# Advaith-Sajeev/LiDAR-Vision-VQA

Measured on AMD Instinct MI355X. Metric: fused tokens/sec/GPU + cross-attn MFMA-roofline % (32k pts x 196 patches), higher is better.
Workload: dtype bf16; 1 GPU; BASELINE configs[1]: 32768-pt scenes (Dist-C) -> hard voxelise (0.1, 0.1, 0.2) T=10 max=60000 + MeanVFE; pillars (0.2, 0.2, 8.0) T=20 max=30000 -> PillarVFE[64] -> PointPillarScatter 512x512 (as an index map; sparse key stream: K|V computed only for the cells with a pillar in their 3x3 neighbourhood, by LayerNorm and the K|V projection folded onto the 64-channel conv token, every other key from th; parallelism=scene-parallel x1

## Files before the change

include/lvq.h:

```cpp
#ifndef LVQ_H
#define LVQ_H

#include <stddef.h>
#include <stdint.h>

#ifdef __cplusplus
extern "C" {
#endif

typedef void *lvq_stream_t;
typedef uint16_t lvq_bf16;

enum {
    LVQ_OK = 0,
    LVQ_EINVAL = -1,
    LVQ_EWORKSPACE = -2,
    LVQ_ELAUNCH = -3,
    LVQ_EOVERFLOW = -4,
    LVQ_EUNSUPPORTED = -5
};

const char *lvq_version(void);
const char *lvq_strerror(int code);

typedef struct lvq_tuning {
    int32_t attn_no32;
    int32_t attn32_nw;
    int32_t attn_pipe;
    int32_t attn_nsplit;
    int32_t attn_qt;
    int32_t attn_nw;
    int32_t gemm_no_gemv;
    int32_t gemm_stream_c_mb;
    int32_t gemm_no256;
    int32_t gemm_no256x256;
    int32_t gemm_256x256_min_tiles;
    int32_t gemm_ln_tiles;
    int32_t pillar_vfe_generic;
    int32_t voxel_path;
    int32_t pairs_one_wg;
    int32_t ca_fused_variant;
    uint64_t ca_fused_stamps;
    int32_t conv_rows_grid;
    int32_t reserved[7];
} lvq_tuning;
void lvq_tuning_defaults(lvq_tuning *t);
int lvq_set_tuning(const lvq_tuning *t);
int lvq_get_tuning(lvq_tuning *t);


int lvq_mask_points_by_range(const float *pts, int64_t n, int c, const float *range_host, uint8_t *keep,
                             lvq_stream_t stream);

size_t lvq_voxelize_hard_workspace_bytes(int64_t n_points, int n_scenes);
int lvq_voxelize_hard(const float *pts, const int32_t *scene_off, int64_t n_points, int n_scenes, int c,
                      const float *range_host, const float *vsize_host, const int32_t *grid_host,
                      int max_pts, int max_voxels, int break_on_cap, int64_t voxel_capacity,
                      float *voxels, int32_t *coords_bzyx, int32_t *num_pts, int32_t *scene_voxel_off,
                      void *ws, size_t ws_bytes, lvq_stream_t stream);

int lvq_voxelize_mean(const float *pts, const int32_t *scene_off, int64_t n_points, int n_scenes, int c,
                      const float *range_host, const float *vsize_host, const int32_t *grid_host, int max_pts,
                      int max_voxels, int64_t voxel_capacity, float *voxel_features, int32_t *coords_bzyx,
                      int32_t *num_pts, int32_t *scene_voxel_off, void *ws, size_t ws_bytes, lvq_stream_t stream);

int lvq_mean_vfe(const float *voxels, const int32_t *num_pts, int64_t m_cap, const int32_t *n_voxels_dev,
                 int t, int c, float *out, lvq_stream_t stream);

int lvq_pillar_vfe(const float *voxels, const int32_t *num_pts, const int32_t *coords_bzyx, int64_t m_cap,
                   const int32_t *n_voxels_dev, int t, int c, int n_layers, const float *const *w_host,
                   const float *const *scale_host, const float *const *shift_host, const int32_t *cin_host,
                   const int32_t *cout_host, int flags, const float *vsize_host, const float *offset_host,
                   float *out, lvq_stream_t stream);

size_t lvq_voxelize_dynamic_workspace_bytes(int64_t n_points, int batch_size, const int32_t *grid_host, int ndim);
int lvq_voxelize_dynamic(const float *pts, int64_t n, int c, int batch_size, const float *range_host,
                         const float *vsize_host, const int32_t *grid_host, int ndim, int32_t *unq_inv,
                         int32_t *pt_coords, int32_t *unq_key, int32_t *unq_cnt, int32_t *coords_bzyx,
                         int32_t *counts, void *ws, size_t ws_bytes, lvq_stream_t stream);

int lvq_voxel_slab_plan(int64_t keyspace, int64_t n, int hard, int *logslab, int *nslabs, int *caps);

int lvq_scatter_mean(const float *pts, int64_t n, int c, int col0, int nc, const int32_t *unq_inv,
                     const int32_t *unq_cnt, int64_t m_cap, float *sums, float *out, lvq_stream_t stream);

int lvq_dynamic_pfn(const float *pts, int64_t n, int c, const int32_t *unq_inv, const int32_t *pt_coords,
                    const float *points_mean, int kind, int n_layers, const float *const *w_host,
                    const float *const *scale_host, const float *const *shift_host, const int32_t *cin_host,
                    const int32_t *cout_host, int flags, const float *vsize_host, const float *offset_host,
                    float *xmax_tmp, float *out, lvq_stream_t stream);

int lvq_pillar_scatter(const float *feat, const int32_t *coords_bzyx, int64_t m_cap, const int32_t *n_voxels_dev,
                       int ch, int batch, int ny, int nx, float *canvas, lvq_stream_t stream);



int lvq_layernorm(const float *x, const float *add, int add_rows, int add_group, const float *gamma,
// ... 239 lines not shown
```

lidar-vision-vqa_amd/_ffi.py:

```python
from __future__ import annotations

import ctypes
import os
import re
from typing import List, Optional, Sequence

import torch

_HERE = os.path.dirname(os.path.abspath(__file__))
LIB_PATH = os.environ.get("LVQ_LIB_PATH") or os.path.join(_HERE, "liblvq_hip.so")
HEADER_PATH = os.path.join(os.path.dirname(_HERE), "include", "lvq.h")

LVQ_OK = 0
LVQ_EUNSUPPORTED = -5


class LvqError(RuntimeError):
    pass


_lib: Optional[ctypes.CDLL] = None


class Tuning(ctypes.Structure):
    _fields_ = [(n, ctypes.c_int32) for n in (
        "attn_no32", "attn32_nw", "attn_pipe", "attn_nsplit", "attn_qt", "attn_nw", "gemm_no_gemv", "gemm_stream_c_mb", "gemm_no256",
        "gemm_no256x256", "gemm_256x256_min_tiles", "gemm_ln_tiles", "pillar_vfe_generic", "voxel_path", "pairs_one_wg",
        "ca_fused_variant")] + [("ca_fused_stamps", ctypes.c_uint64), ("conv_rows_grid", ctypes.c_int32), ("reserved", ctypes.c_int32 * 7)]


TUNING_FIELDS = tuple(n for n, _ in Tuning._fields_ if n != "reserved")


def tuning_from_env(env=None) -> dict:
    e = os.environ if env is None else env

    def flag(name):
        return 1 if e.get(name) else 0

    def num(name):
        return int(e[name]) if e.get(name) else 0

    return {
        "attn_no32": flag("LVQ_ATTN_NO32"), "attn32_nw": num("LVQ_ATTN32_NW"),
        "attn_pipe": -1 if e.get("LVQ_ATTN_NO_PIPE") else flag("LVQ_ATTN_PIPE"),
        "attn_nsplit": num("LVQ_ATTN_NSPLIT"), "attn_qt": num("LVQ_ATTN_QT"), "attn_nw": num("LVQ_ATTN_NW"),
        "gemm_no_gemv": flag("LVQ_GEMM_NO_GEMV"),
        "gemm_stream_c_mb": -1 if e.get("LVQ_GEMM_NO_STREAM_C") else num("LVQ_GEMM_STREAM_C_MB"),
        "gemm_no256": flag("LVQ_GEMM_NO256"), "gemm_no256x256": flag("LVQ_GEMM_NO256X256"),
        "gemm_256x256_min_tiles": num("LVQ_GEMM_256X256_MIN_TILES"), "gemm_ln_tiles": flag("LVQ_GEMM_LN_TILES"),
        "pillar_vfe_generic": flag("LVQ_PILLAR_VFE_GENERIC"),
        "voxel_path": 2 if e.get("LVQ_VOXEL_LEGACY") else flag("LVQ_VOXEL_BINNED"),
        "pairs_one_wg": flag("LVQ_PAIRS_ONE_WG"), "ca_fused_variant": num("LVQ_CA_DBG"), "ca_fused_stamps": 0,
        "conv_rows_grid": 0,
    }


def set_tuning(**fields) -> dict:
    rec = tuning_from_env()
    for k, v in fields.items():
        if k not in TUNING_FIELDS:
            raise LvqError(f"lvq_tuning has no field {k!r}")
        rec[k] = int(v)
    t = Tuning()
    for k, v in rec.items():
        setattr(t, k, v)
    check(lib().lvq_set_tuning(ctypes.byref(t)), "lvq_set_tuning")
    return rec


def get_tuning() -> dict:
    t = Tuning()
    check(lib().lvq_get_tuning(ctypes.byref(t)), "lvq_get_tuning")
    return {k: int(getattr(t, k)) for k in TUNING_FIELDS}


class tuning:

    def __init__(self, **fields):
        self.fields = fields

    def __enter__(self):
        self.old = get_tuning()
        cur = dict(self.old)
        cur.update({k: int(v) for k, v in self.fields.items()})
        _push(cur)
        return self

    def __exit__(self, *exc):
        _push(self.old)
        return False


def _push(rec: dict):
    t = Tuning()
    for k, v in rec.items():
        if k not in TUNING_FIELDS:
            raise LvqError(f"lvq_tuning has no field {k!r}")
        setattr(t, k, v)
    check(lib().lvq_set_tuning(ctypes.byref(t)), "lvq_set_tuning")


_C_TYPES = {"int": ctypes.c_int, "int64_t": ctypes.c_int64, "size_t": ctypes.c_size_t, "float": ctypes.c_float}
_C_RETURNS = dict(_C_TYPES, **{"void": None, "const char *": ctypes.c_char_p})


def prototypes(text: Optional[str] = None) -> dict:
# ... 119 lines not shown
```

lidar-vision-vqa_amd/csrc/bev_tiles.hip:

```cpp
#include "common.h"
#include <type_traits>
#include <utility>

namespace bt {

typedef __attribute__((ext_vector_type(8))) short bf16x8;
typedef __attribute__((ext_vector_type(4))) float f32x4;
typedef __attribute__((ext_vector_type(2))) __bf16 bf16x2_t;
typedef uint32_t u32x4 __attribute__((ext_vector_type(4)));

__device__ __forceinline__ uint32_t pack_bf16(float a, float b) {
    bf16x2_t p = {(__bf16)a, (__bf16)b};
    return *reinterpret_cast<uint32_t *>(&p);
}
typedef _Float16 f16x2_t __attribute__((ext_vector_type(2)));
__device__ __forceinline__ uint32_t pack_f16(float a, float b) {
    f16x2_t p = {(_Float16)a, (_Float16)b};
    return __builtin_bit_cast(uint32_t, p);
}

constexpr int TS = 8, TCELLS = 64;
constexpr int NPIECE = 8, PCELLS = 8;
constexpr int PH = 4, PW = 6, PHALO = PH * PW;
constexpr int NSLOT = NPIECE * PHALO;
// ... 917 lines not shown
                        oh[2 * jj] = pack_bf16(acc[jj][0] * rstd + tv[0], acc[jj][1] * rstd + tv[1]);
                        oh[2 * jj + 1] = pack_bf16(acc[jj][2] * rstd + tv[2], acc[jj][3] * rstd + tv[3]);
                    }
                    if (valid) {
#pragma unroll
                        for (int q = 0; q < 2 * JH; q += 2)
                            *reinterpret_cast<uint2 *>(dst + 2 * (2 * HF * JH + q)) = make_uint2(oh[q], oh[q + 1]);
                    }
                };
                half_out(std::integral_constant<int, 0>{});
                half_out(std::integral_constant<int, 1>{});
            };
            f32x4 te_a[2 * JH], te_b[2 * JH];
            int2 pd_a, pd_b;
            request(0, te_a, pd_a);
            if (has_nx) conv_tile(ih_nx, buf ^ 1);
            request(1, te_b, pd_b);
            emit(0, te_a, pd_a);
            request(2, te_a, pd_a);
            emit(1, te_b, pd_b);
            request(3, te_b, pd_b);
            emit(2, te_a, pd_a);
            emit(3, te_b, pd_b);
        }
        buf ^= 1;
    }
}

struct ConvArgs {
    const float *feat;
    const int32_t *idx;
    const int32_t *live_list;
    const int2 *piece_dirty;
    const int32_t *counts;
    const float *w9, *b9;
    const uint16_t *rh, *rl;
    const float *r0;
    float c0, inv_d, eps;
    int S, H, W;
    uint16_t *th, *tl;
    float *rstd;
    int32_t *key;
};

typedef int i32x2 __attribute__((ext_vector_type(2)));
template <int N> __device__ __forceinline__ void vm_wait() { asm volatile("s_waitcnt vmcnt(%0)" ::"n"(N) : "memory"); }
template <int OFF> __device__ __forceinline__ void vm_load16(f32x4 &d, const void *p) {
    asm volatile("global_load_dwordx4 %0, %1, off offset:%2" : "=&v"(d) : "v"(p), "n"(OFF) : "memory");
}
__device__ __forceinline__ void vm_load8(i32x2 &d, const void *p) { asm volatile("global_load_dwordx2 %0, %1, off" : "=&v"(d) : "v"(p) : "memory"); }
template <class T> __device__ __forceinline__ void vm_load4(T &d, const void *p) {
    static_assert(sizeof(T) == 4, "one dword");
    asm volatile("global_load_dword %0, %1, off" : "=&v"(d) : "v"(p) : "memory");
}
__device__ __forceinline__ void vm_dma16(const void *src, uint32_t dst) {
    uint32_t keep;
    asm volatile("s_mov_b32 %0, m0\n\ts_mov_b32 m0, %2\n\ts_nop 0\n\tglobal_load_lds_dwordx4 %1, off\n\ts_mov_b32 m0, %0"
                 : "=&s"(keep) : "v"(src), "s"(dst) : "memory");
}
template <class T> __device__ __forceinline__ void landed(T &x) { asm volatile("" : "+v"(x)); }
template <int... I, class F> __device__ __forceinline__ void static_for(std::integer_sequence<int, I...>, F &&f) { (f(std::integral_constant<int, I>{}), ...); }
template <int N, class F> __device__ __forceinline__ void static_for(F &&f) { static_for(std::make_integer_sequence<int, N>{}, f); }
__device__ __forceinline__ void lds_barrier() {
    asm volatile("s_waitcnt lgkmcnt(0)" ::: "memory");
    __builtin_amdgcn_s_barrier();
    asm volatile("" ::: "memory");
}

template <bool X3>
__global__ void __launch_bounds__(512) k_conv_rows(ConvArgs a) {
    constexpr int C = 64, NWV = 8, RING = 8;
    extern __shared__ __attribute__((aligned(16))) uint8_t smem[];
    uint16_t *t_hi = reinterpret_cast<uint16_t *>(smem);
    uint16_t *t_lo = t_hi + TCELLS * C;
    float *halo = reinterpret_cast<float *>(t_lo + TCELLS * C);
    int32_t *idxh = reinterpret_cast<int32_t *>(halo + 2 * NSLOT * C);
    int32_t *mcode = idxh + 2 * 256;
    i32x2 *mdirty = reinterpret_cast<i32x2 *>(mcode + RING * NPIECE);
    float *part = reinterpret_cast<float *>(mdirty + RING * NPIECE);
    const int tid = threadIdx.x, lane = tid & 63, wid = tid >> 6, l15 = lane & 15, g4 = lane >> 4;
    const int tw = a.W / TS;
    const int n_live = a.counts[0];
    const int64_t n_groups = ((int64_t)n_live + NPIECE - 1) / NPIECE;
    const int64_t g_begin = blockIdx.x, g_step = gridDim.x;
    if (g_begin >= n_groups) return;
    const int n_my = (int)((n_groups - g_begin + g_step - 1) / g_step);

    float wk[9][8], bk[8];
#pragma unroll
    for (int c = 0; c < 8; ++c) {
        const int ch = (tid & 7) * 8 + c;
        bk[c] = a.b9 ? a.b9[ch] : 0.f;
#pragma unroll
        for (int k = 0; k < 9; ++k) wk[k][c] = a.w9[ch * 9 + k];
    }
    const int rt = wid & 3;
    bf16x8 ra0, ra1, rl0, rl1;
    {
        const uint16_t *rp = a.rh + (16 * rt + l15) * C + 8 * g4;
        ra0 = *reinterpret_cast<const bf16x8 *>(rp);
        ra1 = *reinterpret_cast<const bf16x8 *>(rp + 32);
        rl0 = ra0; rl1 = ra1;
        if (X3) {
            const uint16_t *rpl = a.rl + (16 * rt + l15) * C + 8 * g4;
            rl0 = *reinterpret_cast<const bf16x8 *>(rpl);
            rl1 = *reinterpret_cast<const bf16x8 *>(rpl + 32);
// ... 122 lines not shown
        vm_wait<0>();
        landed(ra0); landed(ra1); landed(rl0); landed(rl1); landed(rinit);
#pragma unroll
        for (int c = 0; c < 8; ++c) {
            landed(bk[c]);
#pragma unroll
            for (int k = 0; k < 9; ++k) landed(wk[k][c]);
        }
        __syncthreads();
        conv_tile(idxh, halo, 0);
        __syncthreads();
        row_sums();
        if (tid < 256) idxh[tid] = k2 ? i2 : -1;
        __syncthreads();
    }
    for (int it = 0; it < n_my; ++it) {
        const int cur = it & 1, nx = cur ^ 1;
        const bool has_nx = it + 1 < n_my;
        dma_halo(idxh + cur * 256, cur);
        bool ok_i, ok_m;
        const int64_t off_i = idx_off(it + 3, ok_i);
        const int64_t k_m = piece_k(it + 4, tid & 7, ok_m);
        int iw, mc;
        i32x2 md;
        vm_load4(iw, a.idx + off_i);
        vm_load4(mc, a.live_list + k_m);
        vm_load8(md, a.piece_dirty + k_m);
        finish_rows(it);
        if (has_nx) conv_tile(idxh + nx * 256, halo + nx * NSLOT * C, it + 1);
        lds_barrier();
        if (has_nx) row_sums();
        vm_wait<0>();
        landed(iw); landed(mc); landed(md);
        if (tid < 256) idxh[nx * 256 + tid] = ok_i ? iw : -1;
        if (tid < NPIECE) {
            const int m = ((it + 4) & (RING - 1)) * NPIECE + tid;
            mcode[m] = ok_m ? mc : -1;
            mdirty[m] = ok_m ? md : i32x2{0, 0};
        }
        lds_barrier();
    }
}

struct KvRowArgs {
    const uint16_t *th, *tl;
    const float *rstd;
    const int32_t *key;
    const int32_t *n_rows;
    const uint16_t *mh, *ml;
    const float *m0;
    const float *te;
    uint16_t *out;
    int k_fp16;
};

template <int J, bool X3, bool TH>
__global__ void __launch_bounds__(512) k_kv_rows(KvRowArgs a) {
    constexpr int N = 128 * J, C = 64, JH = J / 2;
    static_assert(J % 2 == 0, "even J");
    extern __shared__ __attribute__((aligned(16))) uint8_t smem[];
    uint16_t *t_hi = reinterpret_cast<uint16_t *>(smem);
    uint16_t *t_lo = t_hi + 2 * TCELLS * C;
    float *pbias = reinterpret_cast<float *>(t_lo + 2 * TCELLS * C);
    constexpr int SROW = N + 8;
    uint16_t *sbuf = reinterpret_cast<uint16_t *>(pbias + N);
    const int tid = threadIdx.x, lane = tid & 63, wid = tid >> 6, l15 = lane & 15, g4 = lane >> 4;
    const int64_t n_rows = *a.n_rows;
    const int64_t n_groups = (n_rows + TCELLS - 1) / TCELLS;
    const bool x8 = gridDim.x >= 16 && gridDim.x % 16 == 0;
    const int nxcd = x8 ? 8 : 1;
    const int xcd = x8 ? (int)blockIdx.x & 7 : 0;
    const int half = x8 ? ((int)blockIdx.x >> 3) & 1 : (int)blockIdx.x & 1;
    const int wg_r = x8 ? (int)blockIdx.x >> 4 : (int)blockIdx.x >> 1, wg_R = x8 ? (int)gridDim.x >> 4 : ((int)gridDim.x + 1) >> 1;
    const int64_t per_x = (n_groups + nxcd - 1) / nxcd;
    const int64_t x_begin = (int64_t)xcd * per_x, x_end = x_begin + per_x < n_groups ? x_begin + per_x : n_groups;
    const int64_t g_begin = x_begin + wg_r, g_end = x_end, g_step = wg_R;
    const int ncol0 = half * N;
    const bool as_f16 = a.k_fp16 != 0 && half == 0;
    for (int e = tid; e < N; e += 512) pbias[e] = a.m0[ncol0 + e];

    bf16x8 wf[J][2], wfl[X3 ? J : 1][2];
#pragma unroll
    for (int j = 0; j < J; ++j) {
        const int n = ncol0 + 16 * J * wid + (TH ? 32 * (j >> 1) + 8 * (l15 >> 2) + 4 * (j & 1) + (l15 & 3) : 16 * j + l15);
        wf[j][0] = *reinterpret_cast<const bf16x8 *>(a.mh + (int64_t)n * C + 8 * g4);
        wf[j][1] = *reinterpret_cast<const bf16x8 *>(a.mh + (int64_t)n * C + 32 + 8 * g4);
        if (X3) {
            wfl[j][0] = *reinterpret_cast<const bf16x8 *>(a.ml + (int64_t)n * C + 8 * g4);
            wfl[j][1] = *reinterpret_cast<const bf16x8 *>(a.ml + (int64_t)n * C + 32 + 8 * g4);
        }
    }
    const int col0 = 16 * J * wid + (TH ? 8 : 4) * g4;
    auto colj = [&](int j) { return TH ? 32 * (j >> 1) + 4 * (j & 1) : 16 * j; };
    const uint32_t lds_t = (uint32_t)(uintptr_t)((__attribute__((address_space(3))) uint16_t *)t_hi);
    auto stage = [&](int64_t g, int buf) {
        const int row = 8 * wid + (lane >> 3), c = lane & 7;
        int64_t r = g * TCELLS + row;
        r = r < n_rows ? r : n_rows - 1;
        const int64_t so = r * C + ((c ^ ((row >> 1) & 7)) << 3);
        const uint32_t dst = __builtin_amdgcn_readfirstlane(lds_t + (uint32_t)((buf * TCELLS + 8 * wid) * C * 2));
        vm_dma16(a.th + so, dst);
        if (X3) vm_dma16(a.tl + so, dst + 2 * TCELLS * C * 2);
    };
    auto load_t = [&](int buf, int gq, bf16x8 &th0, bf16x8 &th1, bf16x8 &tl0, bf16x8 &tl1) {
        const int row = gq * 16 + l15;
        const int c0 = (g4 ^ ((row >> 1) & 7)) * 8, c1 = ((4 + g4) ^ ((row >> 1) & 7)) * 8;
        th0 = *reinterpret_cast<const bf16x8 *>(t_hi + (buf * TCELLS + row) * C + c0);
        th1 = *reinterpret_cast<const bf16x8 *>(t_hi + (buf * TCELLS + row) * C + c1);
        if (X3) {
            tl0 = *reinterpret_cast<const bf16x8 *>(t_lo + (buf * TCELLS + row) * C + c0);
            tl1 = *reinterpret_cast<const bf16x8 *>(t_lo + (buf * TCELLS + row) * C + c1);
        }
    };
    const uint32_t lds_bias = (uint32_t)(uintptr_t)((__attribute__((address_space(3))) float *)pbias) + 4 * col0;
    auto product = [&](auto hf_tag, const bf16x8 &th0, const bf16x8 &th1, const bf16x8 &tl0, const bf16x8 &tl1, f32x4 (&acc)[JH]) {
        constexpr int HF = decltype(hf_tag)::value;
        uint32_t pb = lds_bias;
        asm volatile("" : "+v"(pb));
#pragma unroll
        for (int jj = 0; jj < JH; ++jj) {
            const int j = HF * JH + jj;
            acc[jj] = *(const __attribute__((address_space(3))) f32x4 *)(pb + 4 * colj(j));
            acc[jj] = __builtin_amdgcn_mfma_f32_16x16x32_bf16(wf[j][0], th0, acc[jj], 0, 0, 0);
            acc[jj] = __builtin_amdgcn_mfma_f32_16x16x32_bf16(wf[j][1], th1, acc[jj], 0, 0, 0);
            if (X3) {
                acc[jj] = __builtin_amdgcn_mfma_f32_16x16x32_bf16(wf[j][0], tl0, acc[jj], 0, 0, 0);
                acc[jj] = __builtin_amdgcn_mfma_f32_16x16x32_bf16(wf[j][1], tl1, acc[jj], 0, 0, 0);
                acc[jj] = __builtin_amdgcn_mfma_f32_16x16x32_bf16(wfl[j][0], th0, acc[jj], 0, 0, 0);
                acc[jj] = __builtin_amdgcn_mfma_f32_16x16x32_bf16(wfl[j][1], th1, acc[jj], 0, 0, 0);
            }
        }
    };
    if (g_begin >= g_end) return;
    constexpr int R = TH ? JH : J;
    constexpr int S = N / 256;
    constexpr int D = X3 ? 2 : 1;
    constexpr int M = 8;
#pragma unroll
    for (int j = 0; j < J; ++j) {
        landed(wf[j][0]);
        landed(wf[j][1]);
        if (X3) { landed(wfl[j][0]); landed(wfl[j][1]); }
    }
    auto load_meta = [&](int64_t g, int (&kq)[4], float (&rq)[4]) {
#pragma unroll
        for (int q = 0; q < 4; ++q) {
            int64_t r = g * TCELLS + q * 16 + l15;
            r = r < n_rows ? r : n_rows - 1;
            vm_load4(kq[q], a.key + r);
            vm_load4(rq[q], a.rstd + r);
        }
    };
    auto meta_landed = [&](int (&kq)[4], float (&rq)[4]) {
#pragma unroll
        for (int q = 0; q < 4; ++q) { landed(kq[q]); landed(rq[q]); }
    };
    auto request = [&](int key, f32x4 (&te)[R]) {
        const char *tep = TH ? reinterpret_cast<const char *>(reinterpret_cast<const uint16_t *>(a.te) + (int64_t)key * (2 * N) + ncol0 + col0)
                             : reinterpret_cast<const char *>(a.te + (int64_t)key * (2 * N) + ncol0 + col0);
        static_for<R>([&](auto i) { vm_load16<64 * decltype(i)::value>(te[decltype(i)::value], tep); });
    };
    int kq[4], kn[4];
    float rq[4], rn[4];
    f32x4 te_a[R], te_b[R];
    load_meta(g_begin, kq, rq);
    stage(g_begin, 0);
    vm_wait<D>();
    meta_landed(kq, rq);
    request(kq[0], te_a);
    vm_wait<R>();
    int buf = 0;
    for (int64_t g = g_begin; g < g_end; g += g_step) {
        const bool first = g == g_begin, full = (g + 1) * TCELLS <= n_rows;
        asm volatile("s_waitcnt lgkmcnt(0)" ::: "memory");
        __builtin_amdgcn_s_barrier();
        asm volatile("" ::: "memory");
        const int64_t gn = g + g_step < g_end ? g + g_step : g;
        stage(gn, buf ^ 1);
        load_meta(gn, kn, rn);
        auto emit = [&](int gq, f32x4 (&te)[R], auto &&wait) {
            bf16x8 th0, th1, tl0, tl1;
            load_t(buf, gq, th0, th1, tl0, tl1);
            const float rs = gq == 0 ? rq[0] : gq == 1 ? rq[1] : gq == 2 ? rq[2] : rq[3];
            uint16_t *sb = sbuf + (gq & 1) * 16 * SROW;
            uint16_t *dst = sb + l15 * SROW + col0;
            auto half_out = [&](auto hf_tag) {
                constexpr int HF = decltype(hf_tag)::value;
                f32x4 acc[JH];
                product(hf_tag, th0, th1, tl0, tl1, acc);
                if constexpr (HF == 0) {
                    wait();
#pragma unroll
                    for (int i = 0; i < R; ++i) landed(te[i]);
                }
                uint32_t oh[2 * JH];
#pragma unroll
                for (int jj = 0; jj < JH; ++jj) {
                    const int j = HF * JH + jj;
                    f32x4 tv;
                    if (TH) {
                        const f16x2_t h0 = __builtin_bit_cast(f16x2_t, __float_as_uint(te[TH ? j >> 1 : 0][2 * (j & 1)]));
                        const f16x2_t h1 = __builtin_bit_cast(f16x2_t, __float_as_uint(te[TH ? j >> 1 : 0][2 * (j & 1) + 1]));
                        tv = f32x4{(float)h0[0], (float)h0[1], (float)h1[0], (float)h1[1]};
                    } else {
                        tv = te[TH ? 0 : j];
                    }
                    if (as_f16) {
                        oh[2 * jj] = pack_f16(acc[jj][0] * rs + tv[0], acc[jj][1] * rs + tv[1]);
                        oh[2 * jj + 1] = pack_f16(acc[jj][2] * rs + tv[2], acc[jj][3] * rs + tv[3]);
                    } else {
                        oh[2 * jj] = pack_bf16(acc[jj][0] * rs + tv[0], acc[jj][1] * rs + tv[1]);
                        oh[2 * jj + 1] = pack_bf16(acc[jj][2] * rs + tv[2], acc[jj][3] * rs + tv[3]);
                    }
                }
#pragma unroll
                for (int jj = 0; jj < JH; ++jj)
                    *reinterpret_cast<uint2 *>(dst + colj(HF * JH + jj)) = make_uint2(oh[2 * jj], oh[2 * jj + 1]);
            };
            half_out(std::integral_constant<int, 0>{});
            half_out(std::integral_constant<int, 1>{});
            asm volatile("s_waitcnt lgkmcnt(0)" ::: "memory");
            __builtin_amdgcn_s_barrier();
            asm volatile("" ::: "memory");
            constexpr int UPR = N / 8;
#pragma unroll
            for (int i = 0; i < S; ++i) {
                const int u = (wid * S + i) * 64 + lane, row = u / UPR, c16 = u - row * UPR;
                const int64_t r = g * TCELLS + gq * 16 + row;
                if (r < n_rows)
                    *reinterpret_cast<u32x4 *>(a.out + r * (2 * N) + ncol0 + c16 * 8) = *reinterpret_cast<const u32x4 *>(sb + row * SROW + c16 * 8);
            }
        };
        auto wait_sr = [&]() { if (full) vm_wait<S + R>(); else vm_wait<R>(); };
        request(kq[1], te_b);
        emit(0, te_a, [&]() {
            if (first) vm_wait<D + M + R>(); else vm_wait<S + D + M + R>();
        });
        request(kq[2], te_a);
        emit(1, te_b, [&]() {
            wait_sr();
            meta_landed(kn, rn);
        });
        request(kq[3], te_b);
        emit(2, te_a, [&]() { wait_sr(); });
        request(kn[0], te_a);
        emit(3, te_b, [&]() { wait_sr(); });
#pragma unroll
        for (int q = 0; q < 4; ++q) { kq[q] = kn[q]; rq[q] = rn[q]; }
        buf ^= 1;
    }
    vm_wait<0>();
}

}

extern "C" size_t lvq_bev_tiles_workspace_bytes(int batch, int ny, int nx) {
    if (batch <= 0 || ny <= 0 || nx <= 0) return 0;
    const int64_t total = (int64_t)batch * (ny / 8) * (nx / 8) * bt::NPIECE;
    return lvq_align((size_t)2 * lvq_cdiv(total, bt::CNT_BLOCK) * sizeof(int32_t)) + lvq_align((size_t)total) + 512;
}

extern "C" int lvq_bev_tiles(const int32_t *idx_map, int batch, int ny, int nx, int force_all, int row_base, int32_t *live_list,
                             int32_t *piece_dirty, int32_t *row_src, int32_t *counts, void *ws, size_t ws_bytes, lvq_stream_t stream) {
    if (batch <= 0 || ny <= 0 || nx <= 0 || row_base < 0 || !live_list || !piece_dirty || !row_src || !counts || (!idx_map && !force_all)) return LVQ_EINVAL;
    if ((ny % bt::TS) || (nx % bt::TS)) return LVQ_EUNSUPPORTED;
    const int64_t total = (int64_t)batch * (ny / bt::TS) * (nx / bt::TS) * bt::NPIECE;
    if ((int64_t)row_base + total * bt::PCELLS > 0x7fffffff || batch > 65535) return LVQ_EUNSUPPORTED;
    if (((uintptr_t)row_src & 15) || ((uintptr_t)piece_dirty & 7) || ((uintptr_t)idx_map & 15)) return LVQ_EUNSUPPORTED;
    const int nb = (int)((total + bt::CNT_BLOCK - 1) / bt::CNT_BLOCK);
    LvqArena arena(ws, ws_bytes);
    int32_t *block_cnt = arena.take<int32_t>((size_t)2 * nb);
    uint8_t *masks = arena.take<uint8_t>((size_t)total);
    if (!arena.ok) return LVQ_EWORKSPACE;
    hipStream_t st = lvq_s(stream);
    hipLaunchKernelGGL(bt::k_piece_count, dim3(nb), dim3(256), 0, st, idx_map, batch, ny, nx, force_all, total, block_cnt, masks);
    hipLaunchKernelGGL(bt::k_piece_compact, dim3(nb), dim3(256), 0, st, idx_map, batch, ny, nx, force_all, total, (const int32_t *)block_cnt,
                       (const uint8_t *)masks, nb, row_base, live_list, reinterpret_cast<int2 *>(piece_dirty), row_src, counts);
    return lvq_launch_status();
}

template <int J> static int launch_tile_kv(const bt::KvArgs &a, bool x3, int64_t cap_tiles, hipStream_t st) {
    const size_t lds = (size_t)2 * 2 * bt::TCELLS * 64 * 2 + (size_t)bt::NSLOT * 64 * 4 + 2 * 256 * 4 + (size_t)2 * 4 * bt::TCELLS * 4 +
                       (size_t)128 * J * 4 + 9 * 64 * 4 + 64 * 4 + 64 * 4 + (size_t)2 * 64 * 64 * 2;
    static LvqLdsOnce once;
    if (!lvq_ensure_lds(once, {(const void *)bt::k_tile_kv<J, false>, (const void *)bt::k_tile_kv<J, true>}, lds)) return LVQ_ELAUNCH;
    int64_t grid = (int64_t)lvq_cu_count();
    if (grid > cap_tiles) grid = cap_tiles;
    grid *= 2;
    if (x3) hipLaunchKernelGGL((bt::k_tile_kv<J, true>), dim3((unsigned)grid), dim3(512), lds, st, a);
    else    hipLaunchKernelGGL((bt::k_tile_kv<J, false>), dim3((unsigned)grid), dim3(512), lds, st, a);
    return lvq_launch_status();
}

template <int J> static int launch_kv_rows(const bt::KvRowArgs &a, bool x3, bool t_f16, int64_t cap_tiles, hipStream_t st) {
    const size_t lds = (size_t)2 * 2 * bt::TCELLS * 64 * 2 + (size_t)128 * J * 4 + (size_t)2 * 16 * (128 * J + 8) * 2;
    static LvqLdsOnce once;
    if (lds > 64 * 1024 && !lvq_ensure_lds(once, {(const void *)bt::k_kv_rows<J, false, false>, (const void *)bt::k_kv_rows<J, true, false>,
                                                   (const void *)bt::k_kv_rows<J, false, true>, (const void *)bt::k_kv_rows<J, true, true>}, lds))
        return LVQ_ELAUNCH;
    int64_t grid = (int64_t)lvq_cu_count();
    if (grid > cap_tiles) grid = cap_tiles;
    grid *= 2;
    if (t_f16) {
        if (x3) hipLaunchKernelGGL((bt::k_kv_rows<J, true, true>), dim3((unsigned)grid), dim3(512), lds, st, a);
        else    hipLaunchKernelGGL((bt::k_kv_rows<J, false, true>), dim3((unsigned)grid), dim3(512), lds, st, a);
    } else {
        if (x3) hipLaunchKernelGGL((bt::k_kv_rows<J, true, false>), dim3((unsigned)grid), dim3(512), lds, st, a);
        else    hipLaunchKernelGGL((bt::k_kv_rows<J, false, false>), dim3((unsigned)grid), dim3(512), lds, st, a);
    }
    return lvq_launch_status();
}

extern "C" size_t lvq_bev_tile_kv_workspace_bytes(int64_t cap_tiles) {
    if (cap_tiles <= 0) return 0;
    LvqSizer z;
    z.take<uint16_t>((size_t)cap_tiles * 64 * 64);
    z.take<uint16_t>((size_t)cap_tiles * 64 * 64);
    z.take<float>((size_t)cap_tiles * 64);
    z.take<int32_t>((size_t)cap_tiles * 64);
    return z.total();
}

extern "C" int lvq_bev_tile_kv(const float *pillar_feat, const int32_t *idx_map, const int32_t *live_list, const int32_t *piece_dirty,
                               const int32_t *counts, int64_t cap_tiles, int batch, int ny, int nx, int c_in, const float *w9, const float *b9,
                               const lvq_bf16 *m, const lvq_bf16 *m_lo, const float *m0, const lvq_bf16 *r, const lvq_bf16 *r_lo, const float *r0,
                               float c0, int d_ln, float eps, const void *t_tiled, int t_f16, int n, int k_fp16, lvq_bf16 *kv, void *ws,
                               size_t ws_bytes, lvq_stream_t stream) {
    if (batch <= 0 || ny <= 0 || nx <= 0 || cap_tiles <= 0 || d_ln <= 0 || !idx_map || !live_list || !piece_dirty || !counts || !w9 || !m || !m0 || !r ||
        !r0 || !t_tiled || !kv)
        return LVQ_EINVAL;
    if ((m_lo == nullptr) != (r_lo == nullptr)) return LVQ_EINVAL;
    if ((k_fp16 || t_f16) && ws == nullptr) return LVQ_EUNSUPPORTED;
    if (c_in != 64 || (ny % 8) || (nx % 8) || (n % 256) || n < 256 || n > 1024) return LVQ_EUNSUPPORTED;
    if (((uintptr_t)pillar_feat | (uintptr_t)m | (uintptr_t)m_lo | (uintptr_t)r | (uintptr_t)r_lo | (uintptr_t)m0 | (uintptr_t)r0 | (uintptr_t)t_tiled |
         (uintptr_t)kv) & 15)
        return LVQ_EUNSUPPORTED;
    bt::KvArgs a;
    a.feat = pillar_feat; a.idx = idx_map; a.live_list = live_list; a.piece_dirty = reinterpret_cast<const int2 *>(piece_dirty); a.counts = counts;
    a.w9 = w9; a.b9 = b9; a.mh = m; a.ml = m_lo; a.m0 = m0; a.rh = r; a.rl = r_lo; a.r0 = r0; a.c0 = c0; a.inv_d = 1.0f / (float)d_ln; a.eps = eps;
    a.te = static_cast<const float *>(t_tiled); a.S = batch; a.H = ny; a.W = nx; a.out = kv;
    hipStream_t st = lvq_s(stream);
    const bool x3 = m_lo != nullptr;
    if (ws != nullptr) {
        LvqArena arena(ws, ws_bytes);
        uint16_t *th = arena.take<uint16_t>((size_t)cap_tiles * 64 * 64);
        uint16_t *tl = arena.take<uint16_t>((size_t)cap_tiles * 64 * 64);
        float *rstd = arena.take<float>((size_t)cap_tiles * 64);
        int32_t *key = arena.take<int32_t>((size_t)cap_tiles * 64);
        if (!arena.ok) return LVQ_EWORKSPACE;
        bt::ConvArgs c;
        c.feat = pillar_feat; c.idx = idx_map; c.live_list = live_list; c.piece_dirty = a.piece_dirty; c.counts = counts; c.w9 = w9; c.b9 = b9;
        c.rh = r; c.rl = r_lo; c.r0 = r0; c.c0 = c0; c.inv_d = a.inv_d; c.eps = eps; c.S = batch; c.H = ny; c.W = nx;
        c.th = th; c.tl = x3 ? tl : nullptr; c.rstd = rstd; c.key = key;
        const size_t lds = (size_t)2 * bt::TCELLS * 64 * 2 + (size_t)2 * bt::NSLOT * 64 * 4 + 2 * 256 * 4 + (size_t)8 * bt::NPIECE * (4 + 8) +
                           (size_t)4 * bt::TCELLS * 4;
        static LvqLdsOnce once;
        if (!lvq_ensure_lds(once, {(const void *)bt::k_conv_rows<false>, (const void *)bt::k_conv_rows<true>}, lds)) return LVQ_ELAUNCH;
        int64_t grid = (int64_t)lvq_cu_count();
        const int hook = lvq_tune().conv_rows_grid;
        if (hook > 0) grid = hook < grid ? hook : grid;
        else if (grid > cap_tiles) grid = cap_tiles;
        if (x3) hipLaunchKernelGGL((bt::k_conv_rows<true>), dim3((unsigned)grid), dim3(512), lds, st, c);
        else    hipLaunchKernelGGL((bt::k_conv_rows<false>), dim3((unsigned)grid), dim3(512), lds, st, c);
        bt::KvRowArgs k;
        k.th = th; k.tl = x3 ? tl : nullptr; k.rstd = rstd; k.key = key; k.n_rows = counts + 2; k.mh = m; k.ml = m_lo; k.m0 = m0; k.te = static_cast<const float *>(t_tiled); k.out = kv; k.k_fp16 = k_fp16;
        switch (n / 128) {
            case 2: return launch_kv_rows<2>(k, x3, t_f16 != 0, cap_tiles, st);
            case 4: return launch_kv_rows<4>(k, x3, t_f16 != 0, cap_tiles, st);
            case 6: return launch_kv_rows<6>(k, x3, t_f16 != 0, cap_tiles, st);
            case 8: return launch_kv_rows<8>(k, x3, t_f16 != 0, cap_tiles, st);
            default: return LVQ_EUNSUPPORTED;
        }
    }
    switch (n / 128) {
        case 2: return launch_tile_kv<2>(a, x3, cap_tiles, st);
        case 4: return launch_tile_kv<4>(a, x3, cap_tiles, st);
        case 6: return launch_tile_kv<6>(a, x3, cap_tiles, st);
        case 8: return launch_tile_kv<8>(a, x3, cap_tiles, st);
        default: return LVQ_EUNSUPPORTED;
    }
}

extern "C" int lvq_bev_scene_pairs(const int32_t *row_src, int batch, int n_tiles, int row_base, int cap_tiles, int32_t *pair_src,
                                   int32_t *pair_info, lvq_stream_t stream) {
    if (!row_src || !pair_src || !pair_info || batch <= 0 || n_tiles <= 0 || cap_tiles <= 0 || row_base < 0) return LVQ_EINVAL;
    if (((uintptr_t)row_src & 15) || (int64_t)n_tiles * bt::TCELLS > 0x7fffffff || batch > 65535) return LVQ_EUNSUPPORTED;
    if (cap_tiles >= n_tiles && cap_tiles >= 2 && !lvq_tune().pairs_one_wg) {
        const int64_t ne = (int64_t)n_tiles * bt::TCELLS;
        int64_t chunk = (ne + 63) / 64;
        chunk = (chunk + 1023) / 1024 * 1024;
        const int nch = (int)((ne + chunk - 1) / chunk);
        hipLaunchKernelGGL(bt::k_scene_pair_count, dim3(nch, batch), dim3(bt::PAIR2_NT), 0, lvq_s(stream), row_src, n_tiles, row_base, cap_tiles, (int)chunk,
                           pair_src);
        hipLaunchKernelGGL(bt::k_scene_pair_write, dim3(nch, batch), dim3(bt::PAIR2_NT), 0, lvq_s(stream), row_src, n_tiles, row_base, cap_tiles, (int)chunk,
                           nch, pair_src, pair_info);
        return lvq_launch_status();
    }
    hipLaunchKernelGGL(bt::k_scene_pairs, dim3(batch), dim3(bt::PAIR_NT), 0, lvq_s(stream), row_src, n_tiles, row_base, cap_tiles, pair_src, pair_info);
    return lvq_launch_status();
}

extern "C" int lvq_bev_shared_lists(const int32_t *row_src, int batch, int n_tiles, int row_base, int cap_tiles, int32_t *list_src, int32_t *list_info,
                                    void *ws, size_t ws_bytes, lvq_stream_t stream) {
    if (!row_src || !list_src || !list_info || batch <= 0 || n_tiles <= 0 || cap_tiles <= 0 || row_base < 0) return LVQ_EINVAL;
    if (((uintptr_t)row_src & 15) || (int64_t)n_tiles * bt::TCELLS > 0x7fffffff || batch > 65534) return LVQ_EUNSUPPORTED;
    if (cap_tiles < n_tiles) return LVQ_EUNSUPPORTED;
    const int ne = n_tiles * bt::TCELLS;
    LvqArena arena(ws, ws_bytes);
    uint8_t *flag = arena.take<uint8_t>((size_t)ne);
    int32_t *cnt = arena.take<int32_t>((size_t)(2 * batch + 1) * 64);
    if (!arena.ok) return LVQ_EWORKSPACE;
    int64_t chunk = ((int64_t)ne + 63) / 64;
    chunk = (chunk + 1023) / 1024 * 1024;
    const int nch = (int)(((int64_t)ne + chunk - 1) / chunk);
    hipStream_t st = lvq_s(stream);
    hipLaunchKernelGGL(bt::k_shared_flags, dim3((unsigned)lvq_cdiv(ne, bt::SH_NT * 4)), dim3(bt::SH_NT), 0, st, row_src, batch, ne, row_base, flag);
    hipLaunchKernelGGL(bt::k_shared_count, dim3(nch, batch), dim3(bt::SH_NT), 0, st, row_src, flag, batch, n_tiles, row_base, (int)chunk, cnt);
    hipLaunchKernelGGL(bt::k_shared_write, dim3(nch, batch + 1), dim3(bt::SH_NT), 0, st, row_src, flag, batch, n_tiles, row_base, cap_tiles, (int)chunk,
                       nch, cnt, list_src, list_info);
    return lvq_launch_status();
}

template <int J> static int launch_tile_tokens(const bt::TokArgs &a, bool x3, bool olo, int64_t cap_tiles, hipStream_t st) {
    const size_t lds = (size_t)2 * 2 * bt::TCELLS * 64 * 2 + (size_t)bt::NSLOT * 64 * 4 + 2 * 256 * 4 + (size_t)2 * 8 * bt::TCELLS * 2 * 4 +
                       (size_t)3 * 128 * J * 4 + 9 * 64 * 4 + 64 * 4;
// ... 37 lines not shown
```

Measured before the change: 1.145 million fused tokens/s.

## Restructure kv_rows pipeline: per-quarter prefetch, fixed column parts, SGPR-based loads

Rewrites the K|V row-projection kernel so each of the four 16-row quarters owns its own prefetch slot. The next group's key, rstd and table-row gathers are issued right after that quarter's outputs are computed, replacing the shared double-buffered metadata and table registers. The output width is now split into fixed 128*J column parts (J=2 or 4), with workgroups looping over parts, so large n no longer needs J=6/8 instantiations. Row loads use scalar-base plus VGPR-offset addressing, and a tuning knob for the grid size is added. Holding four sets of prefetch registers raises register pressure, and the computed vmcnt wait counts are fragile.

```diff
diff --git a/include/lvq.h b/include/lvq.h
--- a/include/lvq.h
+++ b/include/lvq.h
@@ -42,7 +42,8 @@
     int32_t ca_fused_variant;
     uint64_t ca_fused_stamps;
     int32_t conv_rows_grid;
-    int32_t reserved[7];
+    int32_t kv_rows_grid;
+    int32_t reserved[6];
 } lvq_tuning;
 void lvq_tuning_defaults(lvq_tuning *t);
 int lvq_set_tuning(const lvq_tuning *t);
diff --git a/lidar-vision-vqa_amd/_ffi.py b/lidar-vision-vqa_amd/_ffi.py
--- a/lidar-vision-vqa_amd/_ffi.py
+++ b/lidar-vision-vqa_amd/_ffi.py
@@ -26,7 +26,8 @@
     _fields_ = [(n, ctypes.c_int32) for n in (
         "attn_no32", "attn32_nw", "attn_pipe", "attn_nsplit", "attn_qt", "attn_nw", "gemm_no_gemv", "gemm_stream_c_mb", "gemm_no256",
         "gemm_no256x256", "gemm_256x256_min_tiles", "gemm_ln_tiles", "pillar_vfe_generic", "voxel_path", "pairs_one_wg",
-        "ca_fused_variant")] + [("ca_fused_stamps", ctypes.c_uint64), ("conv_rows_grid", ctypes.c_int32), ("reserved", ctypes.c_int32 * 7)]
+        "ca_fused_variant")] + [("ca_fused_stamps", ctypes.c_uint64), ("conv_rows_grid", ctypes.c_int32), ("kv_rows_grid", ctypes.c_int32),
+                                                    ("reserved", ctypes.c_int32 * 6)]
 
 
 TUNING_FIELDS = tuple(n for n, _ in Tuning._fields_ if n != "reserved")
@@ -52,7 +53,7 @@
         "pillar_vfe_generic": flag("LVQ_PILLAR_VFE_GENERIC"),
         "voxel_path": 2 if e.get("LVQ_VOXEL_LEGACY") else flag("LVQ_VOXEL_BINNED"),
         "pairs_one_wg": flag("LVQ_PAIRS_ONE_WG"), "ca_fused_variant": num("LVQ_CA_DBG"), "ca_fused_stamps": 0,
-        "conv_rows_grid": 0,
+        "conv_rows_grid": 0, "kv_rows_grid": 0,
     }
 
 
diff --git a/lidar-vision-vqa_amd/csrc/bev_tiles.hip b/lidar-vision-vqa_amd/csrc/bev_tiles.hip
--- a/lidar-vision-vqa_amd/csrc/bev_tiles.hip
+++ b/lidar-vision-vqa_amd/csrc/bev_tiles.hip
@@ -993,6 +993,10 @@
 template <class T> __device__ __forceinline__ void vm_load4(T &d, const void *p) {
     static_assert(sizeof(T) == 4, "one dword");
     asm volatile("global_load_dword %0, %1, off" : "=&v"(d) : "v"(p) : "memory");
+}
+template <class T> __device__ __forceinline__ void vm_load4s(T &d, const void *base, uint32_t off) {
+    static_assert(sizeof(T) == 4, "one dword");
+    asm volatile("global_load_dword %0, %1, %2" : "=&v"(d) : "v"(off), "s"(base) : "memory");
 }
 __device__ __forceinline__ void vm_dma16(const void *src, uint32_t dst) {
     uint32_t keep;
@@ -1221,31 +1225,31 @@
     const float *te;
     uint16_t *out;
     int k_fp16;
+    int n;
 };
 
+template <int BASE, int S> __device__ __forceinline__ void vm_wait_stores(int ns) {
+    switch (ns) {
+        case 0: vm_wait<BASE>(); break;
+        case 1: vm_wait<BASE + S>(); break;
+        case 2: vm_wait<BASE + 2 * S>(); break;
+        case 3: vm_wait<BASE + 3 * S>(); break;
+        default: vm_wait<BASE + 4 * S>(); break;
+    }
+}
+
 template <int J, bool X3, bool TH>
-__global__ void __launch_bounds__(512) k_kv_rows(KvRowArgs a) {
+__device__ __forceinline__ void kv_rows_part(const KvRowArgs &a, uint8_t *smem, int part, int64_t n_rows, int64_t g_begin, int64_t g_end, int64_t g_step) {
     constexpr int N = 128 * J, C = 64, JH = J / 2;
     static_assert(J % 2 == 0, "even J");
-    extern __shared__ __attribute__((aligned(16))) uint8_t smem[];
     uint16_t *t_hi = reinterpret_cast<uint16_t *>(smem);
     uint16_t *t_lo = t_hi + 2 * TCELLS * C;
     float *pbias = reinterpret_cast<float *>(t_lo + 2 * TCELLS * C);
     constexpr int SROW = N + 8;
     uint16_t *sbuf = reinterpret_cast<uint16_t *>(pbias + N);
     const int tid = threadIdx.x, lane = tid & 63, wid = tid >> 6, l15 = lane & 15, g4 = lane >> 4;
-    const int64_t n_rows = *a.n_rows;
-    const int64_t n_groups = (n_rows + TCELLS - 1) / TCELLS;
-    const bool x8 = gridDim.x >= 16 && gridDim.x % 16 == 0;
-    const int nxcd = x8 ? 8 : 1;
-    const int xcd = x8 ? (int)blockIdx.x & 7 : 0;
-    const int half = x8 ? ((int)blockIdx.x >> 3) & 1 : (int)blockIdx.x & 1;
-    const int wg_r = x8 ? (int)blockIdx.x >> 4 : (int)blockIdx.x >> 1, wg_R = x8 ? (int)gridDim.x >> 4 : ((int)gridDim.x + 1) >> 1;
-    const int64_t per_x = (n_groups + nxcd - 1) / nxcd;
-    const int64_t x_begin = (int64_t)xcd * per_x, x_end = x_begin + per_x < n_groups ? x_begin + per_x : n_groups;
-    const int64_t g_begin = x_begin + wg_r, g_end = x_end, g_step = wg_R;
-    const int ncol0 = half * N;
-    const bool as_f16 = a.k_fp16 != 0 && half == 0;
+    const int ld = 2 * a.n, ncol0 = part * N;
+    const bool as_f16 = a.k_fp16 != 0 && ncol0 + 16 * J * __builtin_amdgcn_readfirstlane(wid) < a.n;
     for (int e = tid; e < N; e += 512) pbias[e] = a.m0[ncol0 + e];
 
     bf16x8 wf[J][2], wfl[X3 ? J : 1][2];
@@ -1300,57 +1304,60 @@
             }
         }
     };
-    if (g_begin >= g_end) return;
     constexpr int R = TH ? JH : J;
     constexpr int S = N / 256;
     constexpr int D = X3 ? 2 : 1;
-    constexpr int M = 8;
+    constexpr int KR = 2;
 #pragma unroll
     for (int j = 0; j < J; ++j) {
         landed(wf[j][0]);
         landed(wf[j][1]);
         if (X3) { landed(wfl[j][0]); landed(wfl[j][1]); }
     }
-    auto load_meta = [&](int64_t g, int (&kq)[4], float (&rq)[4]) {
-#pragma unroll
-        for (int q = 0; q < 4; ++q) {
-            int64_t r = g * TCELLS + q * 16 + l15;
-            r = r < n_rows ? r : n_rows - 1;
-            vm_load4(kq[q], a.key + r);
-            vm_load4(rq[q], a.rstd + r);
-        }
-    };
-    auto meta_landed = [&](int (&kq)[4], float (&rq)[4]) {
-#pragma unroll
-        for (int q = 0; q < 4; ++q) { landed(kq[q]); landed(rq[q]); }
-    };
-    auto request = [&](int key, f32x4 (&te)[R]) {
-        const char *tep = TH ? reinterpret_cast<const char *>(reinterpret_cast<const uint16_t *>(a.te) + (int64_t)key * (2 * N) + ncol0 + col0)
-                             : reinterpret_cast<const char *>(a.te + (int64_t)key * (2 * N) + ncol0 + col0);
+    auto load_row = [&](auto &x, auto *src, int64_t g, int q) {
+        const int64_t last = n_rows - 1 - g * TCELLS;
+        const int lim = last < TCELLS - 1 ? (int)last : TCELLS - 1;
+        int r = q * 16 + l15;
+        asm volatile("" : "+v"(r));
+        vm_load4s(x, src + g * TCELLS, 4u * (uint32_t)(r < lim ? r : lim));
+    };
+    auto t_row = [&](int key) {
+        return TH ? reinterpret_cast<const char *>(reinterpret_cast<const uint16_t *>(a.te) + (int64_t)key * ld + ncol0 + col0)
+                  : reinterpret_cast<const char *>(a.te + (int64_t)key * ld + ncol0 + col0);
+    };
+    auto request = [&](const char *tep, f32x4 (&te)[R]) {
         static_for<R>([&](auto i) { vm_load16<64 * decltype(i)::value>(te[decltype(i)::value], tep); });
     };
-    int kq[4], kn[4];
-    float rq[4], rn[4];
-    f32x4 te_a[R], te_b[R];
-    load_meta(g_begin, kq, rq);
-    stage(g_begin, 0);
-    vm_wait<D>();
-    meta_landed(kq, rq);
-    request(kq[0], te_a);
-    vm_wait<R>();
+    auto next = [&](int64_t g) { return g + g_step < g_end ? g + g_step : g; };
+    int kn[4];
+    float rq[4];
+    f32x4 te[4][R];
+    {
+        int k0[4];
+#pragma unroll
+        for (int q = 0; q < 4; ++q) load_row(k0[q], a.key, g_begin, q);
+        stage(g_begin, 0);
+        vm_wait<0>();
+        static_for<4>([&](auto q_tag) {
+            constexpr int q = decltype(q_tag)::value;
+            landed(k0[q]);
+            load_row(kn[q], a.key, next(g_begin), q);
+            load_row(rq[q], a.rstd, g_begin, q);
+            request(t_row(k0[q]), te[q]);
+        });
+    }
     int buf = 0;
     for (int64_t g = g_begin; g < g_end; g += g_step) {
         const bool first = g == g_begin, full = (g + 1) * TCELLS <= n_rows;
         asm volatile("s_waitcnt lgkmcnt(0)" ::: "memory");
         __builtin_amdgcn_s_barrier();
         asm volatile("" ::: "memory");
-        const int64_t gn = g + g_step < g_end ? g + g_step : g;
+        const int64_t gn = next(g), gf = next(gn);
         stage(gn, buf ^ 1);
-        load_meta(gn, kn, rn);
-        auto emit = [&](int gq, f32x4 (&te)[R], auto &&wait) {
+        auto emit = [&](auto q_tag) {
+            constexpr int gq = decltype(q_tag)::value;
             bf16x8 th0, th1, tl0, tl1;
             load_t(buf, gq, th0, th1, tl0, tl1);
-            const float rs = gq == 0 ? rq[0] : gq == 1 ? rq[1] : gq == 2 ? rq[2] : rq[3];
             uint16_t *sb = sbuf + (gq & 1) * 16 * SROW;
             uint16_t *dst = sb + l15 * SROW + col0;
             auto half_out = [&](auto hf_tag) {
@@ -1358,21 +1365,24 @@
                 f32x4 acc[JH];
                 product(hf_tag, th0, th1, tl0, tl1, acc);
                 if constexpr (HF == 0) {
-                    wait();
-#pragma unroll
-                    for (int i = 0; i < R; ++i) landed(te[i]);
+                    vm_wait_stores<3 * (KR + R) + (gq < 3 ? D : 0), S>((first || gq == 3 ? 0 : 4 - gq) + (full ? gq : 0));
+#pragma unroll
+                    for (int i = 0; i < R; ++i) landed(te[gq][i]);
+                    landed(kn[gq]);
+                    landed(rq[gq]);
                 }
+                const float rs = rq[gq];
                 uint32_t oh[2 * JH];
 #pragma unroll
                 for (int jj = 0; jj < JH; ++jj) {
                     const int j = HF * JH + jj;
                     f32x4 tv;
                     if (TH) {
-                        const f16x2_t h0 = __builtin_bit_cast(f16x2_t, __float_as_uint(te[TH ? j >> 1 : 0][2 * (j & 1)]));
-                        const f16x2_t h1 = __builtin_bit_cast(f16x2_t, __float_as_uint(te[TH ? j >> 1 : 0][2 * (j & 1) + 1]));
+                        const f16x2_t h0 = __builtin_bit_cast(f16x2_t, __float_as_uint(te[gq][TH ? j >> 1 : 0][2 * (j & 1)]));
+                        const f16x2_t h1 = __builtin_bit_cast(f16x2_t, __float_as_uint(te[gq][TH ? j >> 1 : 0][2 * (j & 1) + 1]));
                         tv = f32x4{(float)h0[0], (float)h0[1], (float)h1[0], (float)h1[1]};
                     } else {
-                        tv = te[TH ? 0 : j];
+                        tv = te[gq][TH ? 0 : j];
                     }
                     if (as_f16) {
                         oh[2 * jj] = pack_f16(acc[jj][0] * rs + tv[0], acc[jj][1] * rs + tv[1]);
@@ -1388,6 +1398,10 @@
             };
             half_out(std::integral_constant<int, 0>{});
             half_out(std::integral_constant<int, 1>{});
+            const char *tep = t_row(kn[gq]);
+            load_row(kn[gq], a.key, gf, gq);
+            load_row(rq[gq], a.rstd, gn, gq);
+            request(tep, te[gq]);
             asm volatile("s_waitcnt lgkmcnt(0)" ::: "memory");
             __builtin_amdgcn_s_barrier();
             asm volatile("" ::: "memory");
@@ -1397,28 +1411,32 @@
                 const int u = (wid * S + i) * 64 + lane, row = u / UPR, c16 = u - row * UPR;
                 const int64_t r = g * TCELLS + gq * 16 + row;
                 if (r < n_rows)
-                    *reinterpret_cast<u32x4 *>(a.out + r * (2 * N) + ncol0 + c16 * 8) = *reinterpret_cast<const u32x4 *>(sb + row * SROW + c16 * 8);
+                    *reinterpret_cast<u32x4 *>(a.out + r * ld + ncol0 + c16 * 8) = *reinterpret_cast<const u32x4 *>(sb + row * SROW + c16 * 8);
             }
         };
-        auto wait_sr = [&]() { if (full) vm_wait<S + R>(); else vm_wait<R>(); };
-        request(kq[1], te_b);
-        emit(0, te_a, [&]() {
-            if (first) vm_wait<D + M + R>(); else vm_wait<S + D + M + R>();
-        });
-        request(kq[2], te_a);
-        emit(1, te_b, [&]() {
-            wait_sr();
-            meta_landed(kn, rn);
-        });
-        request(kq[3], te_b);
-        emit(2, te_a, [&]() { wait_sr(); });
-        request(kn[0], te_a);
-        emit(3, te_b, [&]() { wait_sr(); });
-#pragma unroll
-        for (int q = 0; q < 4; ++q) { kq[q] = kn[q]; rq[q] = rn[q]; }
+        static_for<4>(emit);
         buf ^= 1;
     }
     vm_wait<0>();
+}
+
+template <int J, bool X3, bool TH>
+__global__ void __launch_bounds__(512) k_kv_rows(KvRowArgs a) {
+    extern __shared__ __attribute__((aligned(16))) uint8_t smem[];
+    const int64_t n_rows = *a.n_rows;
+    const int64_t n_groups = (n_rows + TCELLS - 1) / TCELLS;
+    const int P = 2 * a.n / (128 * J), grid = (int)gridDim.x, b = (int)blockIdx.x;
+    const bool x8 = grid % (8 * P) == 0;
+    const int nxcd = x8 ? 8 : 1, xcd = x8 ? b & 7 : 0, slot = x8 ? b >> 3 : b;
+    const int part0 = grid < P ? b : slot % P, part_step = grid < P ? grid : P;
+    const int wg_r = grid < P ? 0 : slot / P, wg_R = grid < P ? 1 : (x8 ? grid >> 3 : grid) / P;
+    const int64_t per_x = (n_groups + nxcd - 1) / nxcd;
+    const int64_t x_begin = (int64_t)xcd * per_x, x_end = x_begin + per_x < n_groups ? x_begin + per_x : n_groups;
+    if (x_begin + wg_r >= x_end) return;
+    for (int part = part0; part < P; part += part_step) {
+        if (part != part0) lds_barrier();
+        kv_rows_part<J, X3, TH>(a, smem, part, n_rows, x_begin + wg_r, x_end, wg_R);
+    }
 }
 
 }
@@ -1469,7 +1487,10 @@
         return LVQ_ELAUNCH;
     int64_t grid = (int64_t)lvq_cu_count();
     if (grid > cap_tiles) grid = cap_tiles;
-    grid *= 2;
+    const int parts = 2 * a.n / (128 * J);
+    grid *= parts;
+    const int hook = lvq_tune().kv_rows_grid;
+    if (hook > 0 && hook < grid) grid = hook >= parts ? hook / parts * parts : hook;
     if (t_f16) {
         if (x3) hipLaunchKernelGGL((bt::k_kv_rows<J, true, true>), dim3((unsigned)grid), dim3(512), lds, st, a);
         else    hipLaunchKernelGGL((bt::k_kv_rows<J, false, true>), dim3((unsigned)grid), dim3(512), lds, st, a);
@@ -1532,14 +1553,9 @@
         if (x3) hipLaunchKernelGGL((bt::k_conv_rows<true>), dim3((unsigned)grid), dim3(512), lds, st, c);
         else    hipLaunchKernelGGL((bt::k_conv_rows<false>), dim3((unsigned)grid), dim3(512), lds, st, c);
         bt::KvRowArgs k;
-        k.th = th; k.tl = x3 ? tl : nullptr; k.rstd = rstd; k.key = key; k.n_rows = counts + 2; k.mh = m; k.ml = m_lo; k.m0 = m0; k.te = static_cast<const float *>(t_tiled); k.out = kv; k.k_fp16 = k_fp16;
-        switch (n / 128) {
-            case 2: return launch_kv_rows<2>(k, x3, t_f16 != 0, cap_tiles, st);
-            case 4: return launch_kv_rows<4>(k, x3, t_f16 != 0, cap_tiles, st);
-            case 6: return launch_kv_rows<6>(k, x3, t_f16 != 0, cap_tiles, st);
-            case 8: return launch_kv_rows<8>(k, x3, t_f16 != 0, cap_tiles, st);
-            default: return LVQ_EUNSUPPORTED;
-        }
+        k.th = th; k.tl = x3 ? tl : nullptr; k.rstd = rstd; k.key = key; k.n_rows = counts + 2; k.mh = m; k.ml = m_lo; k.m0 = m0; k.te = static_cast<const float *>(t_tiled); k.out = kv; k.k_fp16 = k_fp16; k.n = n;
+        if (n == 256) return launch_kv_rows<2>(k, x3, t_f16 != 0, cap_tiles, st);
+        return launch_kv_rows<4>(k, x3, t_f16 != 0, cap_tiles, st);
     }
     switch (n / 128) {
         case 2: return launch_tile_kv<2>(a, x3, cap_tiles, st);
```

Result: slower. 1.129 million fused tokens/s (-1.4%).
